# phantomzone-org/poulpy

Hardware: AMD Instinct MI355X
Metric: GGSW external-products/sec (N=2^16, 8 limbs) (higher is better)
Workload: dtype f64; 1 GPU; GLWE(rank 1) x GGSW external product, N=65536, 8 limbs, base2k=12, dnum=8, dsize=1; batch_per_gpu=1024, parallelism=single GPU (no collective), rccl_ranks=0, setup_calls=0

## Files before the change

### poulpy_amd/csrc/device_mid.hpp

```cpp
#pragma once
#include "device_fft.hpp"

namespace pz {

#ifndef PZ_MID_RS
#define PZ_MID_RS 144
#endif
constexpr int kMidRS = PZ_MID_RS;
#ifndef PZ_MID_BR_POST
#define PZ_MID_BR_POST 1
#endif
#ifndef PZ_MID_BR_AVPF
#define PZ_MID_BR_AVPF 1
#endif
#ifndef PZ_MID_STAMP
#define PZ_MID_STAMP 0
#endif
#ifndef PZ_MIDR_HALFKEY
#define PZ_MIDR_HALFKEY 0
#endif
#ifndef PZ_MIDR_SADDR
#define PZ_MIDR_SADDR 1
#endif
#ifndef PZ_MIDR_ILV
#define PZ_MIDR_ILV 1
#endif
#ifndef PZ_MIDR_KR
#define PZ_MIDR_KR 6
#endif

struct MidArgs {
    const cplx* T;
    cplx* T2;
    const cplx* P;
    int npi, npo;
    int nrows, ncols;
    int row_max;
    int ncomp;
    int batch, m1, n_ct;
    const cplx* wL2;
    const cplx* tw12t;
    cplx* dummy;
    int groups;
    int stagger, stagger_mod;
    unsigned perm_mul, perm_add;
    double perm_ysign;
    int log_m1;
    int ds_n;
    unsigned char ds_in[32], ds_row[32], ds_coff[32], ds_cb[32];
    const long long* br_lwe;
    long long br_lwe_bs;
    int br_i0, br_blk, br_rm;
    const cplx* w2n;
    int dbg;
};

template <int CT>
__global__ void __launch_bounds__(CT * 256)
k_mid(MidArgs g) {
    constexpr int M2 = 256;
    constexpr int NC = 16 / CT;
    constexpr int RS = 17 * 16;
    extern __shared__ cplx lds[];
    const int tid = threadIdx.x;
    const long long m = (long long)g.m1 * M2;
    const int row = tid >> 4, o = tid & 15;
    const int ctl = row >> 4, rr = row & 15;
    cplx* rowbuf = lds + row * RS;
    cplx* wl = lds + CT * 16 * RS;
    cplx* twrow = wl + M2;

    const bool xcd_map = (g.m1 & 7) == 0 && (gridDim.x & 7) == 0;
    const int xcd = xcd_map ? (blockIdx.x & 7) : 0;
    const int w = xcd_map ? (blockIdx.x >> 3) : blockIdx.x;
    const int W = xcd_map ? (gridDim.x >> 3) : gridDim.x;
    const int rows_x = xcd_map ? g.m1 / 8 : g.m1;
    const int ntiles = rows_x * g.n_ct;
    if (w >= ntiles) return;
    if (tid < M2) wl[tid] = g.wL2[tid];
    __syncthreads();
    {
        const int k = (blockIdx.x >> 3) % 4;
        for (int i = 0; i < k; ++i) __builtin_amdgcn_s_sleep(127);
    }

    cplx x[16];
    auto tile_q1 = [&](int L) { const int k = L / g.n_ct; return xcd_map ? k * 8 + xcd : k; };
    auto src_ptr = [&](int L) {
        const int Lc = min(L, ntiles - 1);
        const int b_ = min((Lc % g.n_ct) * CT + ctl, g.batch - 1);
        const int r_ = min(rr, g.npi - 1);
        return g.T + ((long long)b_ * g.npi + r_) * m + (long long)tile_q1(Lc) * M2 + o;
    };
    auto in_active = [&](int L) { return L < ntiles && (L % g.n_ct) * CT + ctl < g.batch && rr < g.npi; };

#define PZ_MID_FWD(ACTIVE)                                                                        \
    {                                                                                             \
        if (!(ACTIVE)) {                                                                          \
            _Pragma("unroll") for (int n1 = 0; n1 < 16; ++n1) x[n1] = make_double2(0.0, 0.0);     \
        }                                                                                         \
        Bfly<16, false>::run(x);                                                                  \
        _Pragma("unroll") for (int k1 = 0; k1 < 16; ++k1) {                                       \
            cplx v = x[k1];                                                                       \
            if (k1 > 0) v = cmul(v, wl[o * k1]);                                                  \
            rowbuf[k1 * 17 + o] = v;                                                              \
        }                                                                                         \
        row_sync();                                                                               \
        _Pragma("unroll") for (int oo = 0; oo < 16; ++oo) x[oo] = rowbuf[o * 17 + oo];            \
        Bfly<16, false>::run(x);                                                                  \
        row_sync();                                                                               \
        _Pragma("unroll") for (int k2 = 0; k2 < 16; ++k2) rowbuf[o + 16 * k2] = x[k2];            \
        lds_barrier();                                                                            \
    }

    cplx twn = make_double2(0.0, 0.0);
    {
        const cplx* src = src_ptr(w);
#pragma unroll
        for (int n1 = 0; n1 < 16; ++n1) x[n1] = src[16 * n1];
        twn = g.tw12t[(long long)tile_q1(w) * M2 + (tid & 255)];
    }
    if (tid < M2) twrow[tid] = twn;
    const int vq2 = tid & 255, vcg = tid >> 8;
    const int rot = g.row_max > 0 ? (w % g.row_max) : 0;
    cplx pn[NC];
#define PZ_MID_P0(LT)                                                                                  \
    {                                                                                                  \
        const long long base_ = (long long)tile_q1(min((LT), ntiles - 1)) * g.nrows * g.ncols;         \
        _Pragma("unroll") for (int j = 0; j < NC; ++j)                                                 \
            pn[j] = g.P[(base_ + (long long)rot * g.ncols + min(vcg * NC + j, g.ncomp - 1)) * M2 + vq2];  \
    }
    PZ_MID_P0(w)
    PZ_MID_FWD(in_active(w))

    for (int L = w; L < ntiles; L += W) {
        const int q1 = tile_q1(L);
        const int b = (L % g.n_ct) * CT + ctl;

        {
            const int q2 = tid & 255, cg = tid >> 8;
            cplx acc[CT][NC];
#pragma unroll
            for (int i = 0; i < CT; ++i)
#pragma unroll
                for (int j = 0; j < NC; ++j) acc[i][j] = make_double2(0.0, 0.0);
            const cplx* pp[NC];
#pragma unroll
            for (int j = 0; j < NC; ++j) {
                const int c = min(cg * NC + j, g.ncomp - 1);
                pp[j] = g.P + ((long long)q1 * g.nrows * g.ncols + c) * M2 + q2;
            }
            const long long prow = (long long)g.ncols * M2;
            cplx pb[NC];
#define PZ_LOADROW(DST, IT)                                                                     \
// ... 375 lines not shown
                                acc[i][j].x = __builtin_fma(f[i].x, sv.x, acc[i][j].x);
                                acc[i][j].x = __builtin_fma(-f[i].y, sv.y, acc[i][j].x);
                                acc[i][j].y = __builtin_fma(f[i].x, sv.y, acc[i][j].y);
                                acc[i][j].y = __builtin_fma(f[i].y, sv.x, acc[i][j].y);
                            }
                    }
                } else {
                    for (; it + 1 < nrow; it += 2) {
                        PZ_LOADROW(pb, it + 1)
                        PZ_USEROW(pn, it)
                        PZ_LOADROW(pn, it + 2)
                        PZ_USEROW(pb, it + 1)
                    }
                    if (it < nrow) PZ_USEROW(pn, it)
                }
#undef PZ_BR_FMA
#undef PZ_BR_AV
#undef PZ_BR_KROW
#else
                for (; it + 1 < nrow; it += 2) {
                    PZ_LOADROW(pb, it + 1)
                    PZ_USEROW(pn, it)
                    PZ_LOADROW(pn, it + 2)
                    PZ_USEROW(pb, it + 1)
                }
                if (it < nrow) PZ_USEROW(pn, it)
#endif
            } else {
                for (; it + 3 < nrow; it += 2) {
                    PZ_LOADROW(pb, it + 1)
                    PZ_USEROW(pn, it)
                    PZ_LOADROW(pn, it + 2)
                    PZ_USEROW(pb, it + 1)
                }
                const int left = nrow - it;
                if (left == 3) {
                    PZ_LOADROW(pb, it + 1)
                    PZ_USEROW(pn, it)
                    PZ_LOADROW(pn, it + 2)
                    PZ_USEROW(pb, it + 1)
                    PZ_USEROW(pn, it + 2)
                } else if (left == 2) {
                    PZ_LOADROW(pb, it + 1)
                    PZ_USEROW(pn, it)
                    PZ_USEROW(pb, it + 1)
                } else {
                    PZ_USEROW(pn, it)
                }
            }
#undef PZ_LOADROW
#undef PZ_USEROW
#undef PZ_MID_LOADF
            PZ_STAMP(0)
            lds_barrier();
            PZ_STAMP(1)
#pragma unroll
            for (int i = 0; i < CTt; ++i) {
#pragma unroll
                for (int j = 0; j < NC; ++j) {
                    const int c = cg * NC + j;
                    const int q2o = PERM ? (int)((((g.perm_mul * (unsigned)q1 + g.perm_add) >> g.log_m1) + g.perm_mul * (unsigned)q2) & (unsigned)(M2 - 1)) : q2;
                    lds[((vtg * CTt + i) * NP + c) * RS + q2o] = (c < g.ncomp) ? acc[i][j] : make_double2(0.0, 0.0);
                }
            }
            lds_barrier();
            PZ_STAMP(2)
        }
        PZ_MID_XLOAD(L + W)
        PZ_STAMP(8)
        if (wave_out) {
            PZ_MID_LANE
            const int b = (L % g.n_ct) * CT + ctl;
            cplx u[16];
#pragma unroll
            for (int h = 0; h < 2; ++h)
#pragma unroll
                for (int k2 = 0; k2 < 8; ++k2) u[8 * h + k2] = rowbuf[o + 8 * h + 16 * k2];
            if constexpr (PERM) {
#pragma unroll
                for (int t = 0; t < 16; ++t) u[t].y *= g.perm_ysign;
            }
            if (!(dbgv & 16)) { Bfly<8, true>::run(u); Bfly<8, true>::run(u + 8); }
            row_sync();
#pragma unroll
            for (int h = 0; h < 2; ++h)
#pragma unroll
                for (int oo = 0; oo < 8; ++oo) {
                    cplx v = u[8 * h + oo];
                    const int k1 = o + 8 * h;
                    if (k1 > 0 && oo > 0) v = cmulc(v, wl[oo * k1]);
                    rowbuf[k1 * 9 + oo] = v;
                }
            row_sync();
#pragma unroll
            for (int k1 = 0; k1 < 16; ++k1) u[k1] = rowbuf[k1 * 9 + o];
            if (!(dbgv & 16)) Bfly<16, true>::run(u);
            const bool active = b < g.batch && rr < g.npo;
            cplx* dst = active ? g.T2 + ((long long)b * g.npo + rr) * m + (long long)out_q1(q1) * M2 + o
                               : g.dummy + ((long long)blockIdx.x * (NT / 8) + row) * M2 + o;
#if PZ_MID_STAMP
            asm volatile("s_waitcnt lgkmcnt(0)" ::: "memory");
            __builtin_amdgcn_sched_barrier(0);
            PZ_STAMP(9)
#endif
#pragma unroll
            for (int n1 = 0; n1 < 16; ++n1) if (!(dbgv & 8) || u[n1].x == 1.2345e300) st_stream(dst + 8 * n1, cmulc(u[n1], twrow[o + 8 * n1]));
        }
        PZ_STAMP(3)
        lds_barrier();
        PZ_STAMP(4)
        if (tid0 < M2) twrow[tid0] = twn;
        PZ_MID_P0(L + W)
        PZ_MID_ABUF(L + W)
#if PZ_MID_STAMP
        PZ_STAMP(5)
        asm volatile("s_waitcnt vmcnt(4)" ::: "memory");
        PZ_STAMP(6)
        ++st_tiles;
#endif
        PZ_MID_FWD(L + W)
        PZ_STAMP(7)
    }
#if PZ_MID_STAMP
    if ((tid0 & 63) == 0 && (blockIdx.x == 0 || blockIdx.x == 9 || blockIdx.x == 130 || blockIdx.x == 255))
        printf("STAMP wg %d wave %d tiles %d total %llu | product %llu bar1 %llu accwr %llu xload %llu invc %llu stores %llu bar4 %llu p0 %llu xwait %llu fwd %llu\n",
               (int)blockIdx.x, tid0 >> 6, st_tiles, (unsigned long long)(st_t - st_t0), st_acc[0], st_acc[1], st_acc[2], st_acc[8], st_acc[9], st_acc[3], st_acc[4],
               st_acc[5], st_acc[6], st_acc[7]);
#endif
#undef PZ_STAMP
#undef PZ_MID_FWD
#undef PZ_MID_P0
#undef PZ_MID_ABUF
#undef PZ_MID_XLOAD
#undef PZ_MID_LANE
}

template <int CT, int NP, bool PERM, int NR, int KR, bool HALFIN, bool IN, bool DS = false, bool C2 = false>
__device__ __forceinline__ void mid128r_body(const MidArgs& g) {
    static_assert(!C2 || (!DS && !HALFIN && NP == 16), "two-column passes: the plain 16-slot tile");
    constexpr int M2 = 128, NT = CT * NP * 8;
    constexpr int NC = (NP * M2 / NT) > 4 ? (NP * M2 / NT) : 4;
    constexpr int GC = NP / NC, GT = (NT / M2) / GC, CTt = CT / GT;
    static_assert((NT == 512 || NT == 256) && GC * GT == NT / M2 && CTt * GT == CT && KR >= 3 && KR <= 7 && KR <= NR, "k_mid128r tile shape");
    constexpr int RS = kMidRS;
    extern __shared__ cplx lds[];
    const int tid0 = threadIdx.x;
    const long long m = (long long)g.m1 * M2;
    cplx* wl = lds + CT * NP * RS;
    cplx* twrow2 = wl + M2;
#define PZ_MID_LANE                                                                               \
    const int tid = pz_opaque(tid0);                                                              \
    const int row = tid >> 3, o = tid & 7;                                                        \
    const int ctl = row / NP, rr = row % NP;                                                      \
    cplx* const rowbuf = lds + row * RS;                                                          \
    const int vq2 = tid & (M2 - 1), vcg = (tid / M2) % GC, vtg = (tid / M2) / GC;                 \
    (void)ctl; (void)rr; (void)rowbuf; (void)vq2; (void)vcg; (void)vtg; (void)o;

    const bool xcd_map = (g.m1 & 7) == 0 && (gridDim.x & 7) == 0;
    const int xcd = xcd_map ? (blockIdx.x & 7) : 0;
    const int w = xcd_map ? (blockIdx.x >> 3) : blockIdx.x;
    const int W = xcd_map ? (gridDim.x >> 3) : gridDim.x;
    const int rows_x = xcd_map ? g.m1 / 8 : g.m1;
    const int ntiles = rows_x * g.n_ct;
    if (w >= ntiles) return;
    if (tid0 < M2) wl[tid0] = g.wL2[tid0];
    __syncthreads();
    const int tw_e = (HALFIN && NP == 16) ? ((tid0 >> 6) == 0 ? tid0 : ((tid0 >> 6) == 2 ? tid0 - 64 : -1)) : (tid0 < M2 ? tid0 : -1);
    const bool young = tid0 >= 256;
    if (g.stagger_mod & 1) { if (young) __builtin_amdgcn_s_setprio(1); }
    if (g.stagger_mod & 2) { if (!young) __builtin_amdgcn_s_setprio(1); }
    const int nsleep = ((g.stagger_mod & 4) ? !young : young) ? g.stagger : 0;

    auto vL = [&](int V) { return C2 ? w + (V >> 1) * W : V; };
    auto vcol = [&](int V) { return C2 ? (V & 1) : 0; };
    auto vnext = [&](int V) { return C2 ? V + 1 : V + W; };
    const int V0 = C2 ? 0 : w;
    auto kcol = [&](int slot, int col) { return C2 ? 2 * slot + col : min(slot, g.ncomp - 1); };
    auto tile_q1 = [&](int L) { const int k = L / g.n_ct; return xcd_map ? k * 8 + xcd : k; };
    auto out_q1 = [&](int q1_) { return PERM ? (int)((g.perm_mul * (unsigned)q1_ + g.perm_add) & (unsigned)(g.m1 - 1)) : q1_; };
    auto src_ptr = [&](int L, int ctl, int rr, int o) {
        const int Lc = min(L, ntiles - 1);
        const int b_ = min((Lc % g.n_ct) * CT + ctl, g.batch - 1);
        const int r_ = min(rr, g.npi - 1);
        return g.T + ((long long)b_ * g.npi + r_) * m + (long long)tile_q1(Lc) * M2 + o;
    };
    auto in_active = [&](int L, int ctl, int rr) { return L < ntiles && (L % g.n_ct) * CT + ctl < g.batch && rr < g.npi; };
    constexpr int nrow = NR;
    const int rot = DS ? 0 : w % nrow;

    cplx x[16];
    cplx u[16];
    cplx* dst = nullptr;
    cplx twn = make_double2(0.0, 0.0);
    cplx kr[KR][NC];
#if PZ_MIDR_HALFKEY
#pragma unroll
    for (int i = 0; i < KR; ++i)
#pragma unroll
        for (int j = 0; j < NC; ++j) kr[i][j] = make_double2(1.0, 0.0);
#endif

#define PZ_XGROUP(SRC, G4)                                      \
    { _Pragma("unroll") for (int n1 = 4 * (G4); n1 < 4 * (G4) + 4; ++n1) x[n1] = ld_stream((SRC) + 8 * n1); }
#define PZ_SGROUP(G4)                                        \
    { _Pragma("unroll") for (int n1 = 4 * (G4); n1 < 4 * (G4) + 4; ++n1) st_stream(dst + 8 * n1, u[n1]); }
#define PZ_KGROUP(LT, SLOT)                           \
    if (!(PZ_MIDR_HALFKEY && ((SLOT) & 1))) {                                                          \
        const long long base_ = (long long)tile_q1(min(vL(LT), ntiles - 1)) * g.nrows * g.ncols;     \
        const int kc_ = vcol(LT); (void)kc_;                                                           \
        int r_ = rot + (SLOT);                                                                         \
        r_ -= (r_ >= nrow) ? nrow : 0;                                                                 \
        r_ -= (r_ >= nrow) ? nrow : 0;                                                                 \
        const int krow_ = DS ? (int)g.ds_row[r_] : r_;                                                 \
        if constexpr (!PZ_MIDR_SADDR) {                                                                \
            _Pragma("unroll") for (int j = 0; j < NC; ++j) {                                           \
                const int c_ = DS ? min(vcg * NC + j, max((int)g.ds_cb[r_], 1) - 1) + (int)g.ds_coff[r_] : kcol(vcg * NC + j, kc_); \
                kr[SLOT][j] = g.P[(base_ + (long long)krow_ * g.ncols + c_) * M2 + vq2];               \
            }                                                                                          \
        } else if constexpr (DS) {                                                                     \
            const int cb_ = max((int)g.ds_cb[r_], 1) - 1;                                              \
            const char* rp_ = (const char*)(g.P + (base_ + (long long)krow_ * g.ncols + (int)g.ds_coff[r_]) * M2); \
            _Pragma("unroll") for (int j = 0; j < NC; ++j)                                             \
                kr[SLOT][j] = *(const cplx*)(rp_ + (unsigned)(min(vcg * NC + j, cb_) * M2 + vq2) * 16u); \
        } else {    \
            const char* rp_ = (const char*)(g.P + (base_ + (long long)krow_ * g.ncols) * M2);          \
            _Pragma("unroll") for (int j = 0; j < NC; ++j)                                             \
                kr[SLOT][j] = *(const cplx*)(rp_ + (unsigned)(kcol(vcg * NC + j, kc_) * M2 + vq2) * 16u); \
        }                                                                                              \
    }
#define PZ_MIDR_FWD(LT, STORES)                                                                   \
    {                                                                                             \
        PZ_MID_LANE                                                                               \
        if (STORES) { PZ_SGROUP(0) __builtin_amdgcn_sched_barrier(0); }                           \
        if (PZ_MID_STAMP && STORES) { asm volatile("s_waitcnt vmcnt(4)" ::: "memory"); PZ_STAMP(4) } \
        if constexpr (IN) {                                                                       \
        if (!in_active(vL(LT), ctl, rr)) {                                                        \
            _Pragma("unroll") for (int n1 = 0; n1 < 16; ++n1) x[n1] = make_double2(0.0, 0.0);     \
        }                                                                                         \
        Bfly<16, false>::run(x);                                                                  \
        }                                                                                         \
        __builtin_amdgcn_sched_barrier(0);                                                        \
        if (STORES) { PZ_SGROUP(1) __builtin_amdgcn_sched_barrier(0); }                           \
         \
         \
        if constexpr (IN) _Pragma("unroll") for (int hb = 0; hb < 2; ++hb) {                      \
            cplx tw_[8];                                                                          \
            _Pragma("unroll") for (int k1 = 8 * hb; k1 < 8 * hb + 8; ++k1) tw_[k1 - 8 * hb] = wl[o * k1]; \
            __builtin_amdgcn_sched_barrier(0);                                                    \
            _Pragma("unroll") for (int k1 = 8 * hb; k1 < 8 * hb + 8; ++k1) {                      \
                cplx v = x[k1];                                                                   \
                if (k1 > 0) v = cmul(v, tw_[k1 - 8 * hb]);                                        \
                rowbuf[k1 * 9 + o] = v;                                                           \
            }                                                                                     \
            __builtin_amdgcn_sched_barrier(0);                                                    \
        }                                                                                         \
        if (STORES) { PZ_SGROUP(2) __builtin_amdgcn_sched_barrier(0); }                           \
        if constexpr (IN) {                                                                       \
        row_sync();                                                                               \
        _Pragma("unroll") for (int h = 0; h < 2; ++h) {                                           \
            _Pragma("unroll") for (int oo = 0; oo < 8; ++oo) x[8 * h + oo] = rowbuf[(o + 8 * h) * 9 + oo]; \
        }                                                                                         \
        }                                                                                         \
        __builtin_amdgcn_sched_barrier(0);                                                        \
        if (STORES) { PZ_SGROUP(3) __builtin_amdgcn_sched_barrier(0); }                           \
        PZ_KGROUP(LT, 0)                                                                          \
        __builtin_amdgcn_sched_barrier(0);                                                        \
        if constexpr (IN) Bfly<8, false>::run(x);                                                 \
        __builtin_amdgcn_sched_barrier(0);                                                        \
        PZ_KGROUP(LT, 1)                                                                          \
        __builtin_amdgcn_sched_barrier(0);                                                        \
        if constexpr (IN) Bfly<8, false>::run(x + 8);                                             \
        __builtin_amdgcn_sched_barrier(0);                                                        \
        if constexpr (KR > 3) PZ_KGROUP(LT, 2)                                                    \
        if constexpr (KR > 5) PZ_KGROUP(LT, 4)                                                    \
        __builtin_amdgcn_sched_barrier(0);                                                        \
        if constexpr (IN) {                                                                       \
        row_sync();                                                                               \
        _Pragma("unroll") for (int k2 = 0; k2 < 8; ++k2) rowbuf[o + 16 * k2] = x[k2];             \
        }                                                                                         \
        __builtin_amdgcn_sched_barrier(0);                                                        \
        if constexpr (KR > 4) PZ_KGROUP(LT, 3)                                                    \
        __builtin_amdgcn_sched_barrier(0);                                                        \
        if constexpr (IN) { _Pragma("unroll") for (int k2 = 0; k2 < 8; ++k2) rowbuf[o + 8 + 16 * k2] = x[8 + k2]; } \
        if constexpr (KR > 6) PZ_KGROUP(LT, 5)                                                    \
        if (PZ_MID_STAMP && STORES) { PZ_STAMP(5) }                                               \
        lds_barrier();                                                                            \
    }

    if constexpr (IN) {
        PZ_MID_LANE
        const cplx* src_ = src_ptr(vL(V0), ctl, rr, o);
        PZ_XGROUP(src_, 0) PZ_XGROUP(src_, 1) PZ_XGROUP(src_, 2) PZ_XGROUP(src_, 3)
        if (tw_e >= 0) twrow2[tw_e] = g.tw12t[(long long)out_q1(tile_q1(vL(V0))) * M2 + tw_e];
    }
    int par = 0;
#if PZ_MID_STAMP
    unsigned long long st_acc[8] = {0, 0, 0, 0, 0, 0, 0, 0};
    unsigned long long st_t = 0;
    int st_tiles = 0;
#define PZ_STAMP(i) { const unsigned long long t_ = __builtin_amdgcn_s_memtime(); st_acc[i] += t_ - st_t; st_t = t_; }
#else
#define PZ_STAMP(i)
#endif
    PZ_MIDR_FWD(V0, 0)
#if PZ_MID_STAMP
    st_t = __builtin_amdgcn_s_memtime();
    const unsigned long long st_t0 = st_t;
#endif

    for (int V = V0; vL(V) < ntiles; V = vnext(V), par ^= 1) {
        const int L = vL(V), Vn = vnext(V), Ln = vL(Vn), col = vcol(V);
        (void)col; (void)Ln;
        const int q1 = tile_q1(L);
        {
            PZ_MID_LANE
            const int q2 = vq2, cg = vcg;
            cplx acc[CTt][NC];
#pragma unroll
            for (int i = 0; i < CTt; ++i)
#pragma unroll
                for (int j = 0; j < NC; ++j) acc[i][j] = make_double2(0.0, 0.0);
            const cplx* pp[NC];
#pragma unroll
            for (int j = 0; j < NC; ++j) pp[j] = g.P + ((long long)q1 * g.nrows * g.ncols + (DS ? 0 : kcol(cg * NC + j, col))) * M2 + q2;
            const long long prow = (long long)g.ncols * M2;
            const char* const kbase = (const char*)(g.P + (long long)q1 * g.nrows * g.ncols * M2);
            unsigned koff[NC];
#pragma unroll
            for (int j = 0; j < NC; ++j) koff[j] = (unsigned)(kcol(cg * NC + j, col) * M2 + q2) * 16u;
            const cplx* const avp = lds + vtg * CTt * NP * RS + q2;
            cplx av[2][CTt];
#define PZ_LOADROW(DST, IT)                                                                     \
    if (!(PZ_MIDR_HALFKEY && ((IT) & 1))) {                                                     \
        int r_ = (IT) + rot;                                                                    \
        r_ -= (r_ >= nrow) ? nrow : 0;                                                          \
        r_ -= (r_ >= nrow) ? nrow : 0;                                                          \
        if constexpr (DS && !PZ_MIDR_SADDR) {                                                   \
            const int cb_ = max((int)g.ds_cb[r_], 1) - 1, co_ = (int)g.ds_coff[r_];             \
            const long long ro_ = (long long)g.ds_row[r_] * prow;                               \
            _Pragma("unroll") for (int j = 0; j < NC; ++j) DST[j] = pp[j][ro_ + (long long)(min(cg * NC + j, cb_) + co_) * M2]; \
        } else if constexpr (DS) {    \
            const int cb_ = max((int)g.ds_cb[r_], 1) - 1;                                       \
            const char* rp_ = kbase + ((long long)g.ds_row[r_] * prow + (long long)g.ds_coff[r_] * M2) * 16; \
            _Pragma("unroll") for (int j = 0; j < NC; ++j)                                      \
                DST[j] = *(const cplx*)(rp_ + (unsigned)(min(cg * NC + j, cb_) * M2 + q2) * 16u); \
        } else if constexpr (!PZ_MIDR_SADDR) {                                                  \
            const long long off_ = (long long)r_ * prow;                                        \
            _Pragma("unroll") for (int j = 0; j < NC; ++j) DST[j] = pp[j][off_];                \
        } else {                                                                                \
            const char* rp_ = kbase + (long long)r_ * prow * 16;                                \
            _Pragma("unroll") for (int j = 0; j < NC; ++j) DST[j] = *(const cplx*)(rp_ + koff[j]); \
        }                                                                                       \
    }
#define PZ_AVLOAD(DST, IT)                                                                      \
    {                                                                                           \
        int r_ = (IT) + rot;                                                                    \
        r_ -= (r_ >= nrow) ? nrow : 0;                                                          \
        r_ -= (r_ >= nrow) ? nrow : 0;                                                          \
        const int slot_ = DS ? (int)g.ds_in[r_] : r_;    \
        if constexpr (!PZ_MIDR_SADDR) {                                                         \
            _Pragma("unroll") for (int i = 0; i < CTt; ++i) DST[i] = lds[((vtg * CTt + i) * NP + slot_) * RS + q2]; \
        } else {                                                                                \
            const cplx* ar_ = avp + slot_ * RS;                                                 \
            _Pragma("unroll") for (int i = 0; i < CTt; ++i) DST[i] = ar_[i * NP * RS];          \
        }                                                                                       \
        __builtin_amdgcn_sched_barrier(0);    \
    }
#define PZ_FMAROW(AV, SRC, IT)                                                                  \
    {                                                                                           \
        if constexpr (DS) {                  \
            int r_ = (IT) + rot;                                                                \
            r_ -= (r_ >= nrow) ? nrow : 0;                                                      \
            r_ -= (r_ >= nrow) ? nrow : 0;                                                      \
            const int cbv_ = (int)g.ds_cb[r_];                                                  \
            _Pragma("unroll") for (int j = 0; j < NC; ++j)                                      \
                if (cg * NC + j >= cbv_) SRC[j] = make_double2(0.0, 0.0);                       \
        }                                                                                       \
        _Pragma("unroll") for (int i = 0; i < CTt; ++i) {                                       \
            _Pragma("unroll") for (int j = 0; j < NC; ++j) {                                    \
                acc[i][j].x = __builtin_fma(AV[i].x, SRC[j].x, acc[i][j].x);                    \
                acc[i][j].x = __builtin_fma(-AV[i].y, SRC[j].y, acc[i][j].x);                   \
                acc[i][j].y = __builtin_fma(AV[i].x, SRC[j].y, acc[i][j].y);                    \
                acc[i][j].y = __builtin_fma(AV[i].y, SRC[j].x, acc[i][j].y);                    \
            }                                                                                   \
        }                                                                                       \
        __builtin_amdgcn_sched_barrier(0);                                                      \
    }
            PZ_AVLOAD(av[0], 0)
#pragma unroll
            for (int it = 0; it < NR; ++it) {
                if (it + KR - 1 < NR) PZ_LOADROW(kr[(it + KR - 1) % KR], it + KR - 1)
                if (it + 1 < NR) PZ_AVLOAD(av[(it + 1) & 1], it + 1)
                PZ_FMAROW(av[it & 1], kr[it % KR], it)
            }
#undef PZ_LOADROW
#undef PZ_AVLOAD
#undef PZ_FMAROW
            PZ_STAMP(0)
            lds_barrier();
            PZ_STAMP(1)
            {
                const int q2o = PERM ? (int)((((g.perm_mul * (unsigned)q1 + g.perm_add) >> g.log_m1) + g.perm_mul * (unsigned)q2) & (unsigned)(M2 - 1)) : q2;
                cplx* const wb = lds + (vtg * CTt * NP + cg * NC) * RS + q2o;
                if (C2 || g.ncomp >= NP) {
#pragma unroll
                    for (int i = 0; i < CTt; ++i)
#pragma unroll
                        for (int j = 0; j < NC; ++j) wb[(i * NP + j) * RS] = acc[i][j];
                } else {
#pragma unroll
                    for (int i = 0; i < CTt; ++i)
#pragma unroll
                        for (int j = 0; j < NC; ++j) wb[(i * NP + j) * RS] = (cg * NC + j < g.ncomp) ? acc[i][j] : make_double2(0.0, 0.0);
                }
            }
            lds_barrier();
            PZ_STAMP(2)
        }
#if PZ_MIDR_ILV
        for (int i = 0; i < nsleep; ++i) __builtin_amdgcn_s_sleep(2);
        {
            PZ_MID_LANE
            const int b = (L % g.n_ct) * CT + ctl;
            const cplx* src_ = src_ptr(Ln, ctl, rr, o);
            const cplx* twr = twrow2 + par * M2;
            if constexpr (IN) twn = g.tw12t[(long long)out_q1(tile_q1(min(Ln, ntiles - 1))) * M2 + max(tw_e, 0)];
            if constexpr (IN) { PZ_XGROUP(src_, 0) PZ_XGROUP(src_, 1) }
            __builtin_amdgcn_sched_barrier(0);
#pragma unroll
            for (int h = 0; h < 2; ++h)
#pragma unroll
                for (int k2 = 0; k2 < 8; ++k2) u[8 * h + k2] = rowbuf[o + 8 * h + 16 * k2];
            if constexpr (PERM) {
#pragma unroll
                for (int t = 0; t < 16; ++t) u[t].y *= g.perm_ysign;
            }
            __builtin_amdgcn_sched_barrier(0);
            if constexpr (IN) PZ_XGROUP(src_, 2)
            __builtin_amdgcn_sched_barrier(0);
            Bfly<8, true>::run(u);
            __builtin_amdgcn_sched_barrier(0);
            if constexpr (IN) PZ_XGROUP(src_, 3)
            __builtin_amdgcn_sched_barrier(0);
            Bfly<8, true>::run(u + 8);
            row_sync();
#pragma unroll
            for (int h = 0; h < 2; ++h) {
                const int k1 = o + 8 * h;
                cplx tw_[8];
#pragma unroll
                for (int oo = 1; oo < 8; ++oo) tw_[oo] = wl[oo * k1];
                __builtin_amdgcn_sched_barrier(0);
#pragma unroll
                for (int oo = 0; oo < 8; ++oo) {
                    cplx v = u[8 * h + oo];
                    if (oo > 0) v = cmulc(v, tw_[oo]);
                    rowbuf[k1 * 9 + oo] = v;
                }
                __builtin_amdgcn_sched_barrier(0);
            }
            row_sync();
#pragma unroll
            for (int k1 = 0; k1 < 16; ++k1) u[k1] = rowbuf[k1 * 9 + o];
            __builtin_amdgcn_sched_barrier(0);
            if constexpr (IN) {
                if (!in_active(Ln, ctl, rr)) {
#pragma unroll
                    for (int n1 = 0; n1 < 16; ++n1) x[n1] = make_double2(0.0, 0.0);
                }
                Bfly<16, false>::run(x);
                __builtin_amdgcn_sched_barrier(0);
#pragma unroll
                for (int hb = 0; hb < 2; ++hb) {
                    cplx tw_[8];
#pragma unroll
                    for (int k1 = 8 * hb; k1 < 8 * hb + 8; ++k1) tw_[k1 - 8 * hb] = wl[o * k1];
                    __builtin_amdgcn_sched_barrier(0);
#pragma unroll
                    for (int k1 = 8 * hb; k1 < 8 * hb + 8; ++k1) {
                        cplx v = x[k1];
                        if (k1 > 0) v = cmul(v, tw_[k1 - 8 * hb]);
                        rowbuf[k1 * 9 + o] = v;
                    }
                    __builtin_amdgcn_sched_barrier(0);
                }
            }
            Bfly<16, true>::run(u);
            __builtin_amdgcn_sched_barrier(0);
            cplx twa[8];
#pragma unroll
            for (int n1 = 0; n1 < 8; ++n1) twa[n1] = twr[o + 8 * n1];
            __builtin_amdgcn_sched_barrier(0);
            if constexpr (IN) {
                row_sync();
#pragma unroll
                for (int h = 0; h < 2; ++h) {
#pragma unroll
                    for (int oo = 0; oo < 8; ++oo) x[8 * h + oo] = rowbuf[(o + 8 * h) * 9 + oo];
                }
            }
            __builtin_amdgcn_sched_barrier(0);
#pragma unroll
            for (int n1 = 0; n1 < 8; ++n1) u[n1] = cmulc(u[n1], twa[n1]);
            __builtin_amdgcn_sched_barrier(0);
#pragma unroll
            for (int n1 = 0; n1 < 8; ++n1) twa[n1] = twr[o + 8 * (n1 + 8)];
            __builtin_amdgcn_sched_barrier(0);
            const bool active = b < g.batch && rr < (C2 ? NP : g.npo);
            dst = active ? g.T2 + ((long long)b * g.npo + (C2 ? 2 * rr + col : rr)) * m + (long long)out_q1(q1) * M2 + o
                         : g.dummy + ((long long)blockIdx.x * (NT / 8) + row) * M2 + o;
            PZ_SGROUP(0)
            __builtin_amdgcn_sched_barrier(0);
            if constexpr (IN) Bfly<8, false>::run(x);
            __builtin_amdgcn_sched_barrier(0);
            PZ_SGROUP(1)
            __builtin_amdgcn_sched_barrier(0);
#pragma unroll
            for (int n1 = 0; n1 < 8; ++n1) u[n1 + 8] = cmulc(u[n1 + 8], twa[n1]);
            if constexpr (IN) { if (tw_e >= 0) twrow2[(par ^ 1) * M2 + tw_e] = twn; }
            __builtin_amdgcn_sched_barrier(0);
            PZ_KGROUP(Vn, 0)
            __builtin_amdgcn_sched_barrier(0);
            if constexpr (IN) Bfly<8, false>::run(x + 8);
            __builtin_amdgcn_sched_barrier(0);
            PZ_SGROUP(2)
            PZ_KGROUP(Vn, 1)
            __builtin_amdgcn_sched_barrier(0);
            if constexpr (IN) {
                row_sync();
#pragma unroll
                for (int k2 = 0; k2 < 8; ++k2) rowbuf[o + 16 * k2] = x[k2];
            }
            __builtin_amdgcn_sched_barrier(0);
            PZ_SGROUP(3)
            if constexpr (KR > 3) PZ_KGROUP(Vn, 2)
            __builtin_amdgcn_sched_barrier(0);
            if constexpr (IN) {
#pragma unroll
                for (int k2 = 0; k2 < 8; ++k2) rowbuf[o + 8 + 16 * k2] = x[8 + k2];
            }
            if constexpr (KR > 4) PZ_KGROUP(Vn, 3)
            if constexpr (KR > 5) PZ_KGROUP(Vn, 4)
            if constexpr (KR > 6) PZ_KGROUP(Vn, 5)
            PZ_STAMP(3)
            lds_barrier();
        }
#else
        for (int i = 0; i < nsleep; ++i) __builtin_amdgcn_s_sleep(2);
        {
            PZ_MID_LANE
            const int b = (L % g.n_ct) * CT + ctl;
            const cplx* src_ = src_ptr(Ln, ctl, rr, o);
            const cplx* twr = twrow2 + par * M2;
            if constexpr (IN) twn = g.tw12t[(long long)out_q1(tile_q1(min(Ln, ntiles - 1))) * M2 + max(tw_e, 0)];
            if constexpr (IN) PZ_XGROUP(src_, 0)
            __builtin_amdgcn_sched_barrier(0);
#pragma unroll
            for (int h = 0; h < 2; ++h)
#pragma unroll
                for (int k2 = 0; k2 < 8; ++k2) u[8 * h + k2] = rowbuf[o + 8 * h + 16 * k2];
            if constexpr (PERM) {
#pragma unroll
                for (int t = 0; t < 16; ++t) u[t].y *= g.perm_ysign;
            }
            __builtin_amdgcn_sched_barrier(0);
            if constexpr (IN) PZ_XGROUP(src_, 1)
            __builtin_amdgcn_sched_barrier(0);
            Bfly<8, true>::run(u);
            __builtin_amdgcn_sched_barrier(0);
            if constexpr (IN) PZ_XGROUP(src_, 2)
            __builtin_amdgcn_sched_barrier(0);
            Bfly<8, true>::run(u + 8);
            row_sync();
#pragma unroll
            for (int h = 0; h < 2; ++h) {
                const int k1 = o + 8 * h;
                cplx tw_[8];
#pragma unroll
                for (int oo = 1; oo < 8; ++oo) tw_[oo] = wl[oo * k1];
                __builtin_amdgcn_sched_barrier(0);
#pragma unroll
                for (int oo = 0; oo < 8; ++oo) {
                    cplx v = u[8 * h + oo];
                    if (oo > 0) v = cmulc(v, tw_[oo]);
                    rowbuf[k1 * 9 + oo] = v;
                }
                __builtin_amdgcn_sched_barrier(0);
            }
            if constexpr (IN) PZ_XGROUP(src_, 3)
            __builtin_amdgcn_sched_barrier(0);
            row_sync();
#pragma unroll
            for (int k1 = 0; k1 < 16; ++k1) u[k1] = rowbuf[k1 * 9 + o];
            Bfly<16, true>::run(u);
            __builtin_amdgcn_sched_barrier(0);
#pragma unroll
            for (int hb = 0; hb < 2; ++hb) {
                cplx tw_[8];
#pragma unroll
                for (int n1 = 8 * hb; n1 < 8 * hb + 8; ++n1) tw_[n1 - 8 * hb] = twr[o + 8 * n1];
                __builtin_amdgcn_sched_barrier(0);
#pragma unroll
                for (int n1 = 8 * hb; n1 < 8 * hb + 8; ++n1) u[n1] = cmulc(u[n1], tw_[n1 - 8 * hb]);
                __builtin_amdgcn_sched_barrier(0);
            }
            if constexpr (IN) { if (tw_e >= 0) twrow2[(par ^ 1) * M2 + tw_e] = twn; }
            const bool active = b < g.batch && rr < (C2 ? NP : g.npo);
            dst = active ? g.T2 + ((long long)b * g.npo + (C2 ? 2 * rr + col : rr)) * m + (long long)out_q1(q1) * M2 + o
                         : g.dummy + ((long long)blockIdx.x * (NT / 8) + row) * M2 + o;
        }
        PZ_STAMP(3)
        PZ_MIDR_FWD(Vn, 1)
#endif
        PZ_STAMP(6)
#if PZ_MID_STAMP
        ++st_tiles;
#endif
    }
#if PZ_MID_STAMP
    if ((tid0 & 63) == 0 && (blockIdx.x == 0 || blockIdx.x == 9 || blockIdx.x == 130 || blockIdx.x == 255))
        printf("STAMP wg %d wave %d tiles %d total %llu | product %llu bar1 %llu accwr %llu inv %llu xwait %llu fwd %llu bar6 %llu\n",
               (int)blockIdx.x, tid0 >> 6, st_tiles, (unsigned long long)(st_t - st_t0), st_acc[0], st_acc[1], st_acc[2], st_acc[3], st_acc[4],
               st_acc[5], st_acc[6]);
#endif
#undef PZ_STAMP
#undef PZ_XGROUP
#undef PZ_SGROUP
#undef PZ_KGROUP
#undef PZ_MIDR_FWD
#undef PZ_MID_LANE
}


template <int CT, int NP, bool PERM, int NR, bool HALFIN = false, int KR = ((NP == 32 || CT * NP * 8 == 256) ? 3 : PZ_MIDR_KR), bool DS = false, bool C2 = false>
__global__ void __launch_bounds__(CT * NP * 8)
k_mid128r(MidArgs g) {
    static_assert(!HALFIN || NP >= 16, "HALFIN: 16- and 32-slot tiles");
    static_assert(!DS || !PERM, "digit groups: plain product only");
    if constexpr (HALFIN) {
        if (((threadIdx.x >> 3) % NP) >= NP / 2) {
            mid128r_body<CT, NP, PERM, NR, KR, true, false, DS, C2>(g);
            return;
        }
    }
    mid128r_body<CT, NP, PERM, NR, KR, HALFIN, true, DS, C2>(g);
}



__global__ void __launch_bounds__(256)
k_permute_pmat(const cplx* __restrict__ P, cplx* __restrict__ Pp, int npolys, int m1, int m2) {
    __shared__ cplx tile[16][17];
    const int tx = threadIdx.x & 15, ty = threadIdx.x >> 4;
    const int tiles_q1 = m1 / 16, tiles_q2 = m2 / 16;
    int t = blockIdx.x;
    const int tq1 = t % tiles_q1; t /= tiles_q1;
    const int tq2 = t % tiles_q2; t /= tiles_q2;
    const int p = t;
    const long long m = (long long)m1 * m2;
    tile[ty][tx] = P[(long long)p * m + (long long)(tq2 * 16 + ty) * m1 + tq1 * 16 + tx];
    __syncthreads();
    Pp[((long long)(tq1 * 16 + ty) * npolys + p) * m2 + tq2 * 16 + tx] = tile[tx][ty];
}

template <bool CONJ>
__global__ void __launch_bounds__(256)
k_permute_pmat_gal(const cplx* __restrict__ P, cplx* __restrict__ Pp, int npolys, int m1, unsigned mul, unsigned add, unsigned mul_inv) {
    constexpr int M2 = 128;
    __shared__ cplx tile[M2][17];
    const int tiles_q1 = m1 / 16;
    const int tq1 = blockIdx.x % tiles_q1, p = blockIdx.x / tiles_q1;
    const unsigned m = (unsigned)m1 * M2;
    const cplx* src = P + (long long)p * m + tq1 * 16;
#pragma unroll
    for (int i = 0; i < 8; ++i) {
        const int e = threadIdx.x + 256 * i;
        tile[e >> 4][e & 15] = src[(long long)(e >> 4) * m1 + (e & 15)];
    }
    __syncthreads();
#pragma unroll
    for (int i = 0; i < 8; ++i) {
        const int e = threadIdx.x + 256 * i;
        const int q2d = e & (M2 - 1), ql = e >> 7;
        const unsigned q1 = (unsigned)(tq1 * 16 + ql);
        const unsigned q1d = (mul_inv * (q1 - add)) & (unsigned)(m1 - 1);
        const unsigned q = (mul * (q1d + (unsigned)m1 * (unsigned)q2d) + add) & (m - 1u);
        cplx v = tile[q / (unsigned)m1][ql];
        if (CONJ) v.y = -v.y;
        Pp[((long long)q1d * npolys + p) * M2 + q2d] = v;
    }
}

}
```

Before: 98620 external-products/s.

## Replace per-tile div/mod indexing with incremental tile walker and wave-uniform address math

Introduces a MidWalk iterator that advances (k, g, col) incrementally instead of recomputing L / n_ct and L % n_ct each tile. Source and destination addresses are split into a wave-uniform base plus a precomputed 32-bit lane offset, and the per-lane bounds checks are hoisted into ballot-based wave-uniform fast paths. A separate first-iteration FMA ordering is added in the accumulate macro. The intent is to cut scalar/vector integer ALU work and register pressure in the mid-stage FFT kernel's address computation. The cost is extra complexity, and correctness now relies on the clamping and validity semantics of the walker.

```diff
diff --git a/poulpy_amd/csrc/device_mid.hpp b/poulpy_amd/csrc/device_mid.hpp
--- a/poulpy_amd/csrc/device_mid.hpp
+++ b/poulpy_amd/csrc/device_mid.hpp
@@ -1,5 +1,6 @@
 #pragma once
 #include "device_fft.hpp"
+#include "mid_walk.hpp"
 
 namespace pz {
 
@@ -681,10 +682,12 @@
     const int tid = pz_opaque(tid0);                                                              \
     const int row = tid >> 3, o = tid & 7;                                                        \
     const int ctl = row / NP, rr = row % NP;                                                      \
-    cplx* const rowbuf = lds + row * RS;                                                          \
+    cplx* const rowbuf = lds + row_rs;    \
     const int vq2 = tid & (M2 - 1), vcg = (tid / M2) % GC, vtg = (tid / M2) / GC;                 \
     (void)ctl; (void)rr; (void)rowbuf; (void)vq2; (void)vcg; (void)vtg; (void)o;
 
+    const int row_rs = (tid0 >> 3) * RS;
+    const int wb_rs = (((tid0 / M2) / GC) * CTt * NP + ((tid0 / M2) % GC) * NC) * RS;
     const bool xcd_map = (g.m1 & 7) == 0 && (gridDim.x & 7) == 0;
     const int xcd = xcd_map ? (blockIdx.x & 7) : 0;
     const int w = xcd_map ? (blockIdx.x >> 3) : blockIdx.x;
@@ -700,20 +703,24 @@
     if (g.stagger_mod & 2) { if (!young) __builtin_amdgcn_s_setprio(1); }
     const int nsleep = ((g.stagger_mod & 4) ? !young : young) ? g.stagger : 0;
 
-    auto vL = [&](int V) { return C2 ? w + (V >> 1) * W : V; };
-    auto vcol = [&](int V) { return C2 ? (V & 1) : 0; };
-    auto vnext = [&](int V) { return C2 ? V + 1 : V + W; };
-    const int V0 = C2 ? 0 : w;
+    MidWalk wk = mid_walk_start(w, W, g.n_ct, rows_x, C2);
+    const int wrow0 = __builtin_amdgcn_readfirstlane(tid0 >> 3) & ~7;
+    const int ctl_s = wrow0 / NP, rr0 = wrow0 % NP;
     auto kcol = [&](int slot, int col) { return C2 ? 2 * slot + col : min(slot, g.ncomp - 1); };
-    auto tile_q1 = [&](int L) { const int k = L / g.n_ct; return xcd_map ? k * 8 + xcd : k; };
+    auto tile_q1c = [&](const MidTile& t) { return mid_walk_q1(mid_walk_k_clamped(wk, t), xcd_map, xcd); };
     auto out_q1 = [&](int q1_) { return PERM ? (int)((g.perm_mul * (unsigned)q1_ + g.perm_add) & (unsigned)(g.m1 - 1)) : q1_; };
-    auto src_ptr = [&](int L, int ctl, int rr, int o) {
-        const int Lc = min(L, ntiles - 1);
-        const int b_ = min((Lc % g.n_ct) * CT + ctl, g.batch - 1);
-        const int r_ = min(rr, g.npi - 1);
-        return g.T + ((long long)b_ * g.npi + r_) * m + (long long)tile_q1(Lc) * M2 + o;
+    auto src_base = [&](const MidTile& t) {
+        const int b_ = min(mid_walk_g_clamped(wk, t) * CT + ctl_s, g.batch - 1);
+        return (const char*)(g.T + ((long long)b_ * g.npi * m + (long long)tile_q1c(t) * M2));
     };
-    auto in_active = [&](int L, int ctl, int rr) { return L < ntiles && (L % g.n_ct) * CT + ctl < g.batch && rr < g.npi; };
+    auto tile_in = [&](const MidTile& t) { return t.valid && t.g * CT + ctl_s < g.batch; };
+    const int npo_eff = C2 ? NP : g.npo;
+    const bool all_in = __builtin_amdgcn_ballot_w64(rr0 + ((tid0 >> 3) & 7) >= g.npi) == 0;
+    const bool all_out = __builtin_amdgcn_ballot_w64(rr0 + ((tid0 >> 3) & 7) >= npo_eff) == 0;
+    const int lg_row = g.log_m1 + 11;
+    const unsigned src_lo = ((unsigned)min(rr0 + ((tid0 >> 3) & 7), g.npi - 1) << lg_row) + (unsigned)(tid0 & 7) * 16u;
+    auto dst_lo_of = [&](int rr_, int o_) { return ((unsigned)(C2 ? 2 * rr_ : rr_) << lg_row) + (unsigned)o_ * 16u; };
+    auto key_pts = [&](const MidTile& t) { return (long long)tile_q1c(t) * g.nrows * g.ncols; };
     constexpr int nrow = NR;
     const int rot = DS ? 0 : w % nrow;
 
@@ -729,14 +736,14 @@
         for (int j = 0; j < NC; ++j) kr[i][j] = make_double2(1.0, 0.0);
 #endif
 
-#define PZ_XGROUP(SRC, G4)                                      \
-    { _Pragma("unroll") for (int n1 = 4 * (G4); n1 < 4 * (G4) + 4; ++n1) x[n1] = ld_stream((SRC) + 8 * n1); }
+#define PZ_XGROUP(SRC, G4)          \
+    { _Pragma("unroll") for (int n1 = 4 * (G4); n1 < 4 * (G4) + 4; ++n1) x[n1] = ld_stream((const cplx*)((SRC) + src_lo_) + 8 * n1); }
 #define PZ_SGROUP(G4)                                        \
     { _Pragma("unroll") for (int n1 = 4 * (G4); n1 < 4 * (G4) + 4; ++n1) st_stream(dst + 8 * n1, u[n1]); }
-#define PZ_KGROUP(LT, SLOT)                           \
+#define PZ_KGROUP(KQ, COL, SLOT)   \
     if (!(PZ_MIDR_HALFKEY && ((SLOT) & 1))) {                                                          \
-        const long long base_ = (long long)tile_q1(min(vL(LT), ntiles - 1)) * g.nrows * g.ncols;     \
-        const int kc_ = vcol(LT); (void)kc_;                                                           \
+        const long long base_ = (KQ);                                                                  \
+        const int kc_ = (COL); (void)kc_;                                                              \
         int r_ = rot + (SLOT);                                                                         \
         r_ -= (r_ >= nrow) ? nrow : 0;                                                                 \
         r_ -= (r_ >= nrow) ? nrow : 0;                                                                 \
@@ -760,11 +767,14 @@
 #define PZ_MIDR_FWD(LT, STORES)                                                                   \
     {                                                                                             \
         PZ_MID_LANE                                                                               \
+        const long long kq_ = key_pts(LT);                                                        \
         if (STORES) { PZ_SGROUP(0) __builtin_amdgcn_sched_barrier(0); }                           \
         if (PZ_MID_STAMP && STORES) { asm volatile("s_waitcnt vmcnt(4)" ::: "memory"); PZ_STAMP(4) } \
         if constexpr (IN) {                                                                       \
-        if (!in_active(vL(LT), ctl, rr)) {                                                        \
-            _Pragma("unroll") for (int n1 = 0; n1 < 16; ++n1) x[n1] = make_double2(0.0, 0.0);     \
+        if (!(tile_in(LT) && all_in)) {    \
+            if (!(tile_in(LT) && rr < g.npi)) {                                                   \
+                _Pragma("unroll") for (int n1 = 0; n1 < 16; ++n1) x[n1] = make_double2(0.0, 0.0); \
+            }                                                                                     \
         }                                                                                         \
         Bfly<16, false>::run(x);                                                                  \
         }                                                                                         \
@@ -792,35 +802,35 @@
         }                                                                                         \
         __builtin_amdgcn_sched_barrier(0);                                                        \
         if (STORES) { PZ_SGROUP(3) __builtin_amdgcn_sched_barrier(0); }                           \
-        PZ_KGROUP(LT, 0)                                                                          \
+        PZ_KGROUP(kq_, (LT).col, 0)                                                                          \
         __builtin_amdgcn_sched_barrier(0);                                                        \
         if constexpr (IN) Bfly<8, false>::run(x);                                                 \
         __builtin_amdgcn_sched_barrier(0);                                                        \
-        PZ_KGROUP(LT, 1)                                                                          \
+        PZ_KGROUP(kq_, (LT).col, 1)                                                                          \
         __builtin_amdgcn_sched_barrier(0);                                                        \
         if constexpr (IN) Bfly<8, false>::run(x + 8);                                             \
         __builtin_amdgcn_sched_barrier(0);                                                        \
-        if constexpr (KR > 3) PZ_KGROUP(LT, 2)                                                    \
-        if constexpr (KR > 5) PZ_KGROUP(LT, 4)                                                    \
+        if constexpr (KR > 3) PZ_KGROUP(kq_, (LT).col, 2)                                                    \
+        if constexpr (KR > 5) PZ_KGROUP(kq_, (LT).col, 4)                                                    \
         __builtin_amdgcn_sched_barrier(0);                                                        \
         if constexpr (IN) {                                                                       \
         row_sync();                                                                               \
         _Pragma("unroll") for (int k2 = 0; k2 < 8; ++k2) rowbuf[o + 16 * k2] = x[k2];             \
         }                                                                                         \
         __builtin_amdgcn_sched_barrier(0);                                                        \
-        if constexpr (KR > 4) PZ_KGROUP(LT, 3)                                                    \
+        if constexpr (KR > 4) PZ_KGROUP(kq_, (LT).col, 3)                                                    \
         __builtin_amdgcn_sched_barrier(0);                                                        \
         if constexpr (IN) { _Pragma("unroll") for (int k2 = 0; k2 < 8; ++k2) rowbuf[o + 8 + 16 * k2] = x[8 + k2]; } \
-        if constexpr (KR > 6) PZ_KGROUP(LT, 5)                                                    \
+        if constexpr (KR > 6) PZ_KGROUP(kq_, (LT).col, 5)                                                    \
         if (PZ_MID_STAMP && STORES) { PZ_STAMP(5) }                                               \
         lds_barrier();                                                                            \
     }
 
     if constexpr (IN) {
-        PZ_MID_LANE
-        const cplx* src_ = src_ptr(vL(V0), ctl, rr, o);
+        const char* src_ = src_base(wk.cur);
+        const unsigned src_lo_ = (unsigned)pz_opaque((int)src_lo);
         PZ_XGROUP(src_, 0) PZ_XGROUP(src_, 1) PZ_XGROUP(src_, 2) PZ_XGROUP(src_, 3)
-        if (tw_e >= 0) twrow2[tw_e] = g.tw12t[(long long)out_q1(tile_q1(vL(V0))) * M2 + tw_e];
+        if (tw_e >= 0) twrow2[tw_e] = g.tw12t[(long long)out_q1(tile_q1c(wk.cur)) * M2 + tw_e];
     }
     int par = 0;
 #if PZ_MID_STAMP
@@ -831,16 +841,17 @@
 #else
 #define PZ_STAMP(i)
 #endif
-    PZ_MIDR_FWD(V0, 0)
+    PZ_MIDR_FWD(wk.cur, 0)
 #if PZ_MID_STAMP
     st_t = __builtin_amdgcn_s_memtime();
     const unsigned long long st_t0 = st_t;
 #endif
 
-    for (int V = V0; vL(V) < ntiles; V = vnext(V), par ^= 1) {
-        const int L = vL(V), Vn = vnext(V), Ln = vL(Vn), col = vcol(V);
-        (void)col; (void)Ln;
-        const int q1 = tile_q1(L);
+    for (; wk.cur.valid; mid_walk_step(wk), par ^= 1) {
+        const MidTile Tc = wk.cur, Tn = wk.next;
+        const int col = Tc.col;
+        (void)col;
+        const int q1 = mid_walk_q1(Tc.k, xcd_map, xcd);
         {
             PZ_MID_LANE
             const int q2 = vq2, cg = vcg;
@@ -905,6 +916,21 @@
             _Pragma("unroll") for (int j = 0; j < NC; ++j)                                      \
                 if (cg * NC + j >= cbv_) SRC[j] = make_double2(0.0, 0.0);                       \
         }                                                                                       \
+        if ((IT) == 0) {    \
+             \
+            _Pragma("unroll") for (int i = 0; i < CTt; ++i) {                                   \
+                _Pragma("unroll") for (int j = 0; j < NC; ++j) {                                \
+                    acc[i][j].x = __builtin_fma(AV[i].x, SRC[j].x, acc[i][j].x);                \
+                    acc[i][j].y = __builtin_fma(AV[i].x, SRC[j].y, acc[i][j].y);                \
+                }                                                                               \
+            }                                                                                   \
+            _Pragma("unroll") for (int i = 0; i < CTt; ++i) {                                   \
+                _Pragma("unroll") for (int j = 0; j < NC; ++j) {                                \
+                    acc[i][j].x = __builtin_fma(-AV[i].y, SRC[j].y, acc[i][j].x);               \
+                    acc[i][j].y = __builtin_fma(AV[i].y, SRC[j].x, acc[i][j].y);                \
+                }                                                                               \
+            }                                                                                   \
+        } else                                                                                  \
         _Pragma("unroll") for (int i = 0; i < CTt; ++i) {                                       \
             _Pragma("unroll") for (int j = 0; j < NC; ++j) {                                    \
                 acc[i][j].x = __builtin_fma(AV[i].x, SRC[j].x, acc[i][j].x);                    \
@@ -930,7 +956,7 @@
             PZ_STAMP(1)
             {
                 const int q2o = PERM ? (int)((((g.perm_mul * (unsigned)q1 + g.perm_add) >> g.log_m1) + g.perm_mul * (unsigned)q2) & (unsigned)(M2 - 1)) : q2;
-                cplx* const wb = lds + (vtg * CTt * NP + cg * NC) * RS + q2o;
+                cplx* const wb = lds + wb_rs + q2o;
                 if (C2 || g.ncomp >= NP) {
 #pragma unroll
                     for (int i = 0; i < CTt; ++i)
@@ -950,10 +976,14 @@
         for (int i = 0; i < nsleep; ++i) __builtin_amdgcn_s_sleep(2);
         {
             PZ_MID_LANE
-            const int b = (L % g.n_ct) * CT + ctl;
-            const cplx* src_ = src_ptr(Ln, ctl, rr, o);
+            const int b = Tc.g * CT + ctl_s;
+            const char* src_ = src_base(Tn);
+            const long long kq_n = key_pts(Tn);
+            (void)kq_n;
+            const unsigned src_lo_ = (unsigned)pz_opaque((int)src_lo);
+            (void)src_lo_;
             const cplx* twr = twrow2 + par * M2;
-            if constexpr (IN) twn = g.tw12t[(long long)out_q1(tile_q1(min(Ln, ntiles - 1))) * M2 + max(tw_e, 0)];
+            if constexpr (IN) twn = *(const cplx*)((const char*)(g.tw12t + (long long)out_q1(tile_q1c(Tn)) * M2) + (unsigned)pz_opaque(max(tw_e, 0) * 16));
             if constexpr (IN) { PZ_XGROUP(src_, 0) PZ_XGROUP(src_, 1) }
             __builtin_amdgcn_sched_barrier(0);
 #pragma unroll
@@ -993,9 +1023,11 @@
             for (int k1 = 0; k1 < 16; ++k1) u[k1] = rowbuf[k1 * 9 + o];
             __builtin_amdgcn_sched_barrier(0);
             if constexpr (IN) {
-                if (!in_active(Ln, ctl, rr)) {
-#pragma unroll
-                    for (int n1 = 0; n1 < 16; ++n1) x[n1] = make_double2(0.0, 0.0);
+                if (!(tile_in(Tn) && all_in)) {
+                    if (!(tile_in(Tn) && rr < g.npi)) {
+#pragma unroll
+                        for (int n1 = 0; n1 < 16; ++n1) x[n1] = make_double2(0.0, 0.0);
+                    }
                 }
                 Bfly<16, false>::run(x);
                 __builtin_amdgcn_sched_barrier(0);
@@ -1035,9 +1067,11 @@
 #pragma unroll
             for (int n1 = 0; n1 < 8; ++n1) twa[n1] = twr[o + 8 * (n1 + 8)];
             __builtin_amdgcn_sched_barrier(0);
-            const bool active = b < g.batch && rr < (C2 ? NP : g.npo);
-            dst = active ? g.T2 + ((long long)b * g.npo + (C2 ? 2 * rr + col : rr)) * m + (long long)out_q1(q1) * M2 + o
-                         : g.dummy + ((long long)blockIdx.x * (NT / 8) + row) * M2 + o;
+            dst = (cplx*)((const char*)(g.T2 + (((long long)b * g.npo + (C2 ? col : 0)) * m + (long long)out_q1(q1) * M2)) + dst_lo_of(rr, o));
+            if (!(b < g.batch && all_out)) {
+                const int row_ = pz_opaque(row);
+                if (!(b < g.batch && rr < npo_eff)) dst = g.dummy + ((long long)blockIdx.x * (NT / 8) + row_) * M2 + o;
+            }
             PZ_SGROUP(0)
             __builtin_amdgcn_sched_barrier(0);
             if constexpr (IN) Bfly<8, false>::run(x);
@@ -1048,12 +1082,12 @@
             for (int n1 = 0; n1 < 8; ++n1) u[n1 + 8] = cmulc(u[n1 + 8], twa[n1]);
             if constexpr (IN) { if (tw_e >= 0) twrow2[(par ^ 1) * M2 + tw_e] = twn; }
             __builtin_amdgcn_sched_barrier(0);
-            PZ_KGROUP(Vn, 0)
+            PZ_KGROUP(kq_n, Tn.col, 0)
             __builtin_amdgcn_sched_barrier(0);
             if constexpr (IN) Bfly<8, false>::run(x + 8);
             __builtin_amdgcn_sched_barrier(0);
             PZ_SGROUP(2)
-            PZ_KGROUP(Vn, 1)
+            PZ_KGROUP(kq_n, Tn.col, 1)
             __builtin_amdgcn_sched_barrier(0);
             if constexpr (IN) {
                 row_sync();
@@ -1062,15 +1096,15 @@
             }
             __builtin_amdgcn_sched_barrier(0);
             PZ_SGROUP(3)
-            if constexpr (KR > 3) PZ_KGROUP(Vn, 2)
+            if constexpr (KR > 3) PZ_KGROUP(kq_n, Tn.col, 2)
             __builtin_amdgcn_sched_barrier(0);
             if constexpr (IN) {
 #pragma unroll
                 for (int k2 = 0; k2 < 8; ++k2) rowbuf[o + 8 + 16 * k2] = x[8 + k2];
             }
-            if constexpr (KR > 4) PZ_KGROUP(Vn, 3)
-            if constexpr (KR > 5) PZ_KGROUP(Vn, 4)
-            if constexpr (KR > 6) PZ_KGROUP(Vn, 5)
+            if constexpr (KR > 4) PZ_KGROUP(kq_n, Tn.col, 3)
+            if constexpr (KR > 5) PZ_KGROUP(kq_n, Tn.col, 4)
+            if constexpr (KR > 6) PZ_KGROUP(kq_n, Tn.col, 5)
             PZ_STAMP(3)
             lds_barrier();
         }
@@ -1078,10 +1112,14 @@
         for (int i = 0; i < nsleep; ++i) __builtin_amdgcn_s_sleep(2);
         {
             PZ_MID_LANE
-            const int b = (L % g.n_ct) * CT + ctl;
-            const cplx* src_ = src_ptr(Ln, ctl, rr, o);
+            const int b = Tc.g * CT + ctl_s;
+            const char* src_ = src_base(Tn);
+            const long long kq_n = key_pts(Tn);
+            (void)kq_n;
+            const unsigned src_lo_ = (unsigned)pz_opaque((int)src_lo);
+            (void)src_lo_;
             const cplx* twr = twrow2 + par * M2;
-            if constexpr (IN) twn = g.tw12t[(long long)out_q1(tile_q1(min(Ln, ntiles - 1))) * M2 + max(tw_e, 0)];
+            if constexpr (IN) twn = *(const cplx*)((const char*)(g.tw12t + (long long)out_q1(tile_q1c(Tn)) * M2) + (unsigned)pz_opaque(max(tw_e, 0) * 16));
             if constexpr (IN) PZ_XGROUP(src_, 0)
             __builtin_amdgcn_sched_barrier(0);
 #pragma unroll
@@ -1134,12 +1172,14 @@
                 __builtin_amdgcn_sched_barrier(0);
             }
             if constexpr (IN) { if (tw_e >= 0) twrow2[(par ^ 1) * M2 + tw_e] = twn; }
-            const bool active = b < g.batch && rr < (C2 ? NP : g.npo);
-            dst = active ? g.T2 + ((long long)b * g.npo + (C2 ? 2 * rr + col : rr)) * m + (long long)out_q1(q1) * M2 + o
-                         : g.dummy + ((long long)blockIdx.x * (NT / 8) + row) * M2 + o;
+            dst = (cplx*)((const char*)(g.T2 + (((long long)b * g.npo + (C2 ? col : 0)) * m + (long long)out_q1(q1) * M2)) + dst_lo_of(rr, o));
+            if (!(b < g.batch && all_out)) {
+                const int row_ = pz_opaque(row);
+                if (!(b < g.batch && rr < npo_eff)) dst = g.dummy + ((long long)blockIdx.x * (NT / 8) + row_) * M2 + o;
+            }
         }
         PZ_STAMP(3)
-        PZ_MIDR_FWD(Vn, 1)
+        PZ_MIDR_FWD(Tn, 1)
 #endif
         PZ_STAMP(6)
 #if PZ_MID_STAMP
diff --git a/poulpy_amd/csrc/mid_walk.hpp b/poulpy_amd/csrc/mid_walk.hpp
--- /dev/null
+++ b/poulpy_amd/csrc/mid_walk.hpp
@@ -0,0 +1,54 @@
+#pragma once
+
+#if defined(__HIPCC__)
+#define PZ_WALK_FN __host__ __device__ __forceinline__
+#else
+#define PZ_WALK_FN inline
+#endif
+
+namespace pz {
+
+struct MidTile {
+    int k, g;
+    int col;
+    bool valid;
+};
+
+struct MidWalk {
+    int n_ct, rows;
+    int dk, dg;
+    bool c2;
+    MidTile cur, next;
+};
+
+PZ_WALK_FN int mid_walk_q1(int k, bool xcd_map, int xcd) { return xcd_map ? k * 8 + xcd : k; }
+
+PZ_WALK_FN MidTile mid_walk_after(const MidWalk& s, const MidTile& t) {
+    MidTile n = t;
+    if (s.c2 && t.col == 0) { n.col = 1; return n; }
+    n.col = 0;
+    n.k = t.k + s.dk;
+    n.g = t.g + s.dg;
+    if (n.g >= s.n_ct) { n.g -= s.n_ct; n.k += 1; }
+    n.valid = n.k < s.rows;
+    return n;
+}
+
+PZ_WALK_FN MidWalk mid_walk_start(int w, int W, int n_ct, int rows, bool c2) {
+    MidWalk s;
+    s.n_ct = n_ct; s.rows = rows; s.c2 = c2;
+    s.dk = W / n_ct; s.dg = W % n_ct;
+    s.cur.k = w / n_ct; s.cur.g = w % n_ct; s.cur.col = 0; s.cur.valid = s.cur.k < rows;
+    s.next = mid_walk_after(s, s.cur);
+    return s;
+}
+
+PZ_WALK_FN void mid_walk_step(MidWalk& s) {
+    s.cur = s.next;
+    s.next = mid_walk_after(s, s.cur);
+}
+
+PZ_WALK_FN int mid_walk_k_clamped(const MidWalk& s, const MidTile& t) { return t.valid ? t.k : s.rows - 1; }
+PZ_WALK_FN int mid_walk_g_clamped(const MidWalk& s, const MidTile& t) { return t.valid ? t.g : s.n_ct - 1; }
+
+}
```

Result: no change. 98580 external-products/s (-0.0%).
